# South-Twilight/ParallelWaveGAN

Hardware: AMD Instinct MI355X
Metric: audio samples/sec/GPU (24 kHz PWG, 80-band mel) + RTF at 1/2/4/8 MI355X (higher is better)
Workload: dtype f32 (fp16 hi+lo pair operands, 3 f16 MFMAs per product, fp32 accumulate); 1 GPU; libritts_v1 generator inference, 32 ragged utterances per GPU per step; model=ParallelWaveGANGenerator, hop=300, global_batch=32, frames_per_gpu=24295, parallelism=1 process, 1 GPU (no collective)

## Files before the change

### parallelwavegan_amd/csrc/pwg_capi.hip

```cpp
#include <hip/hip_runtime.h>

#include <algorithm>
#include <cmath>
#include <cstdio>
#include <cstdlib>
#include <cstring>
#include <map>
#include <mutex>
#include <string>
#include <utility>
#include <vector>

#include "../../include/pwg.h"
#include "pwg_internal.h"

#ifndef PWG_SMALL_SPREAD
#define PWG_SMALL_SPREAD 1
#endif

using namespace pwg;

namespace {

thread_local std::string g_err;
// ... 954 lines not shown
      give_back();
      return e;
    }
    h->records.push_back({bucket, a, b});
    return e;
  };

  int* range_flag = (int*)(ws + p->ws_flag);
  hipError_t e = hipSuccess;
  const int pipe_wg = h->n_cu / 8 * 8;
  const bool use_pipe = p->pipe_ok && h->layer_kernel == 3 && p->Tpad <= h->pipe_max && pipe_wg >= h->L;
  const bool split = h->layer_kernel == 2 || h->layer_kernel == 3;
  const bool split16 = h->layer_kernel == 3;
  const bool fuse_first = split16 && h->fuse_first && h->L > 1;
  UttDesc* d_utts = (UttDesc*)(ws + p->ws_utts);
  int* d_tile_utt = (int*)(ws + p->ws_tile_utt);
  long long* d_gap_col0 = (long long*)(ws + p->ws_gap);
  BlockDesc* d_blocks = (BlockDesc*)(ws + p->ws_blocks);
  for (int u0 = 0; u0 < p->n_utts; u0 += PLAN_CHUNK) {
    PlanDescArgs da;
    da.n = std::min(PLAN_CHUNK, p->n_utts - u0);
    da.u0 = u0;
    da.gap_tiles = (int)(h->gap / TILE);
    for (int i = 0; i < da.n; ++i) da.utts[i] = p->utts[u0 + i];
    da.d_utts = d_utts; da.tile_utt = d_tile_utt; da.gap_col0 = d_gap_col0; da.blocks = d_blocks;
    da.zero = u0 == 0 ? sched_ctr : nullptr;
    da.n_zero = (int)((p->ws_flag + sizeof(int) - p->ws_ctr) / sizeof(int));
    da.prog = use_pipe ? (int*)(ws + p->ws_prog) : nullptr;
    da.zx[0] = fuse_first ? reinterpret_cast<unsigned*>(x0) : nullptr;
    da.zx[1] = fuse_first ? reinterpret_cast<unsigned*>(x1) : nullptr;
    da.zx[2] = fuse_first && use_pipe ? reinterpret_cast<unsigned*>(ws + p->ws_x2) : nullptr;
    e = launch_plan_desc(da, p->max_blocks_per_utt, s);
    if (e != hipSuccess) return hip_fail(e, "plan descriptor launch");
  }
  ConvInArgs ca;
  ca.mel = mel; ca.mean = mean; ca.scale = scale; ca.w = packed + h->off_conv_in; ca.c1 = c1;
  ca.wfrag = packed + h->off_conv_in_frag;
  ca.utts = d_utts; ca.n_utts = p->n_utts; ca.F_total = p->F_total; ca.A = h->A; ca.KW = h->KW;
  ca.ctx = h->cfg.aux_context_window; ca.layout = p->layout; ca.use_conv_in = h->cfg.use_conv_in;
  e = timed(PWG_KERNEL_CONV_IN, [&] { return launch_conv_in(ca, s); });
  if (e != hipSuccess) return hip_fail(e, "conv_in launch");

  AuxProjArgs pa;
  pa.c1 = c1; pa.waux = packed + h->off_waux; pa.d = dproj; pa.F_total = p->F_total; pa.A = h->A; pa.GR = h->GR;
  pa.split = split16 ? 2 : split ? 1 : 0;
  pa.split_scale_a = (float)SPLIT_GATE_SCALE_TANH;
// ... 501 lines not shown
```

### parallelwavegan_amd/csrc/pwg_internal.h

```cpp
#pragma once
#include <hip/hip_runtime.h>
#include <stdint.h>

namespace pwg {

constexpr int TILE = 128;
constexpr int KC = 16;
constexpr int MAX_SCALES = 8;
constexpr int AUX_J4 = 8;
constexpr int AUX_MAX_NFWG = 16;

struct UttDesc {
  long long seg_base;
  long long first_tile;
  long long T;
  long long frame_base;
  long long frames;
  long long mel_off;
  long long io_off;
};

struct ConvInArgs {
  const float* mel;
  const float* mean;
// ... 63 lines not shown
  int R, RS, S, SS, KS;
  int dil;
  int nka;
  int nfwg;
  int tap_center;
  int first;
  const float* hw1;
  const float* hw2;
  const float* hb2;
  float* out;
  long long out_stride_t, out_stride_o;
  int O;
  float skip_scale;
};

struct BlockDesc {
  int col;
  int t0;
  int T;
  int frames;
  int frame_base;
  int io_off;
  int utt;
  int pad;
};

struct PersistArgs {
  const float* x_in;
  float* x_out;
  float* skip;
  const float* d;
  const float* tab;
  const BlockDesc* blocks;
  const float* wgp;
  const float* w2;
  const float* bg;
  const float* hw1;
  const float* hw2;
  const float* hb2;
  float* out;
  int tab_left, tab_right, tab_small;
  int H, J1, TL, TR, Fmin, nka;
  int n_blocks;
  int R, RS, S, SS, KS, dil, tap_center, first, O;
  int out_stride_t, out_stride_o;
  float skip_scale;
  int* ctr;
// ... 51 lines not shown
  unsigned* x[2];
  int* ctr;
  int l0, L;
  int half;
  int force_abort;
  int force_timeout;
  int waves_mid;
  int dil[PIPE_MAX_LAYERS];
};

constexpr int SCHED_CTR_STRIDE = 32;

int set_error(int code, const char* msg);

hipError_t allow_lds(const void* kfn, int lds);

constexpr int PLAN_CHUNK = 48;
constexpr int GAP_TILES_MAX = 1 << 20;
struct PlanDescArgs {
  UttDesc utts[PLAN_CHUNK];
  int n;
  int u0;
  int gap_tiles;
  UttDesc* d_utts;
  int* tile_utt;
  long long* gap_col0;
  BlockDesc* blocks;
  int* zero;
  int n_zero;
  int* prog;
  unsigned* zx[3];
};
hipError_t launch_plan_desc(const PlanDescArgs& a, long long max_blocks, hipStream_t s);

hipError_t launch_conv_in(const ConvInArgs& a, hipStream_t s);
hipError_t launch_aux_proj(const AuxProjArgs& a, int layers, hipStream_t s);
hipError_t launch_first_conv(const FirstConvArgs& a, long long n_tiles, hipStream_t s);
hipError_t launch_layer(const LayerArgs& a, int mt, int m2t, bool last, long long n_tiles, hipStream_t s);
hipError_t launch_first_conv_split(const FirstConvArgs& a, long long n_tiles, hipStream_t s);
hipError_t launch_first_conv_split16(const FirstConvArgs& a, long long n_tiles, hipStream_t s);
hipError_t launch_layer_split16(const SplitArgs& a, bool last, int tap_center, int waves_per_wg, int n_wg,
                                hipStream_t s, bool half = false);
hipError_t launch_layer_split(const SplitArgs& a, bool last, int tap_center, int waves_per_wg, int n_wg,
                              hipStream_t s);
hipError_t launch_pipe_split16(const PipeArgs& p, int tap_center, int n_wg, hipStream_t s);
hipError_t launch_sync_split16(const SyncArgs& p, int tap_center, int n_wg, hipStream_t s);
// ... 99 lines not shown
```

### parallelwavegan_amd/csrc/pwg_kernels.hip

```cpp
#include "pwg_internal.h"
#include "../../include/pwg.h"

namespace pwg {

typedef float f32x16 __attribute__((ext_vector_type(16)));
typedef float f32x4 __attribute__((ext_vector_type(4)));

__device__ __forceinline__ long long floordiv(long long a, long long b) {
  long long q = a / b;
  if ((a % b != 0) && (a < 0)) --q;
  return q;
}

__device__ __forceinline__ int find_utt_by_frame(const UttDesc* utts, int n, long long g) {
  int lo = 0, hi = n - 1;
  while (lo < hi) {
    int mid = (lo + hi + 1) >> 1;
    if (utts[mid].frame_base <= g) lo = mid; else hi = mid - 1;
  }
  return lo;
}

template <int OGMAX>
__global__ void __launch_bounds__(256) pwg_conv_in_kernel(const ConvInArgs a) {
// ... 833 lines not shown
      }
    }

    if (nblk < 0) break;
    blk = nblk;
    nblk = ticket_resolve(ticket);
  }
}

__global__ void __launch_bounds__(256) pwg_plan_desc_kernel(const PlanDescArgs a) {
  const int y = blockIdx.y;
  const UttDesc& d = a.utts[y];
  const long long j = (long long)blockIdx.x * 256 + threadIdx.x;
  const long long nb = (d.T + TILE - 1) / TILE * (TILE / 32);
  if (j < nb) {
    BlockDesc b;
    b.t0 = (int)(32 * j);
    b.col = (int)(d.seg_base + b.t0);
    b.T = (int)d.T;
    b.frames = (int)d.frames;
    b.frame_base = (int)d.frame_base;
    b.io_off = (int)d.io_off;
    b.utt = a.u0 + y;
    b.pad = 0;
    a.blocks[d.first_tile * (TILE / 32) + j] = b;
    if (a.prog != nullptr) a.prog[d.first_tile * (TILE / 32) + j] = 0;
    if ((j & (TILE / 32 - 1)) == 0) a.tile_utt[d.first_tile + j / (TILE / 32)] = a.u0 + y;
  }
  if (j < a.gap_tiles) {
    const long long seg_end = d.seg_base + (d.T + TILE - 1) / TILE * TILE;
    a.gap_col0[(long long)(a.u0 + y + 1) * a.gap_tiles + j] = seg_end + j * TILE;
    if (a.u0 == 0 && y == 0) a.gap_col0[j] = j * TILE;
  }
  if (j == 0) a.d_utts[a.u0 + y] = d;
  if (a.zero != nullptr && blockIdx.x == 0 && y == 0)
    for (int i = threadIdx.x; i < a.n_zero; i += 256) a.zero[i] = 0;
  if (a.zx[0] != nullptr && blockIdx.x == 0) {
    const long long seg_end = d.seg_base + (d.T + TILE - 1) / TILE * TILE;
    const int lead = a.u0 == 0 && y == 0 ? a.gap_tiles : 0;
    const int n4 = 64 * TILE / 4;
    typedef unsigned u32x4z __attribute__((ext_vector_type(4)));
    for (int t = 0; t < a.gap_tiles + lead; ++t) {
      const long long col0 = t < a.gap_tiles ? seg_end + (long long)t * TILE : (long long)(t - a.gap_tiles) * TILE;
#pragma unroll
      for (int pl = 0; pl < 3; ++pl) {
        if (a.zx[pl] == nullptr) continue;
        u32x4z* z = reinterpret_cast<u32x4z*>(a.zx[pl] + (size_t)col0 * 64);
// ... 112 lines not shown
```

### parallelwavegan_amd/csrc/pwg_split16.hip

```cpp
#include "pwg_internal.h"


namespace pwg {

namespace {

typedef float f32x4 __attribute__((ext_vector_type(4)));
typedef _Float16 f16x8 __attribute__((ext_vector_type(8)));
typedef unsigned u32x4 __attribute__((ext_vector_type(4)));

__device__ __forceinline__ f32x4 mma16(u32x4 a, u32x4 b, f32x4 c) {
  return __builtin_amdgcn_mfma_f32_16x16x32_f16(__builtin_bit_cast(f16x8, a), __builtin_bit_cast(f16x8, b), c, 0, 0,
                                                0);
}

__device__ __forceinline__ float gate16(float u, float v) {
  u = fminf(u, 64.f);
  const float e1 = __builtin_amdgcn_exp2f(u);
  const float e2 = __builtin_amdgcn_exp2f(v);
  return (1.f - e1) * __builtin_amdgcn_rcpf((1.f + e1) * (1.f + e2));
}

template <int NOPS>
__device__ __forceinline__ void split8x(const float (&v)[8], u32x4& hi, u32x4& lo) {
// ... 36 lines not shown
      "v_fma_mix_f32 %3, %22, %16, %3 op_sel:[1,0,0] op_sel_hi:[1,0,0]\n\t"
      "v_fma_mix_f32 %4, %23, %16, %4 op_sel_hi:[1,0,0]\n\t"
      "v_fma_mix_f32 %5, %23, %16, %5 op_sel:[1,0,0] op_sel_hi:[1,0,0]\n\t"
      "v_fma_mix_f32 %6, %24, %16, %6 op_sel_hi:[1,0,0]\n\t"
      "v_fma_mix_f32 %7, %24, %16, %7 op_sel:[1,0,0] op_sel_hi:[1,0,0]\n\t"
      "s_nop 1"
      : "=&v"(o[0]), "=&v"(o[1]), "=&v"(o[2]), "=&v"(o[3]), "=&v"(o[4]), "=&v"(o[5]), "=&v"(o[6]), "=&v"(o[7])
      : "v"(l[0]), "v"(l[1]), "v"(l[2]), "v"(l[3]), "v"(b0[0]), "v"(b0[1]), "v"(b0[2]), "v"(b0[3]), "v"(c),
        "v"(b1[0]), "v"(b1[1]), "v"(b1[2]), "v"(b1[3]), "v"(h[0]), "v"(h[1]), "v"(h[2]), "v"(h[3]));
}

struct Pair16 {
  unsigned hi, lo;
};
__device__ __forceinline__ Pair16 split_pair16(float v0, float v1) {
  typedef _Float16 f16x2 __attribute__((ext_vector_type(2)));
  const _Float16 h0 = (_Float16)v0, h1 = (_Float16)v1;
  const _Float16 l0 = (_Float16)(v0 - (float)h0), l1 = (_Float16)(v1 - (float)h1);
  return {__builtin_bit_cast(unsigned, f16x2{h0, h1}), __builtin_bit_cast(unsigned, f16x2{l0, l1})};
}

}

__device__ __forceinline__ size_t row16(int c, int g) {
  return (size_t)(c >> 5) * 2048 + (size_t)((c >> 4) & 1) * 1024 + (size_t)g * 64 + (size_t)(c & 15) * 4;
}

__device__ __forceinline__ unsigned row16_bytes(int c, int g) { return (unsigned)row16(c, g) * 4u; }

__device__ __forceinline__ __amdgpu_buffer_rsrc_t rsrc16(const void* base) {
  const unsigned long long b = (unsigned long long)base;
  const unsigned lo = __builtin_amdgcn_readfirstlane((unsigned)b), hi = __builtin_amdgcn_readfirstlane((unsigned)(b >> 32));
  return __builtin_amdgcn_make_buffer_rsrc((void*)(((unsigned long long)hi << 32) | lo), 0, 0x7fffffff, 0x00020000);
}
constexpr int AUX_SC1 = 16;
__device__ __forceinline__ u32x4 ld16_sc1(__amdgpu_buffer_rsrc_t r, unsigned off) {
  return __builtin_bit_cast(u32x4, __builtin_amdgcn_raw_buffer_load_b128(r, off, 0, AUX_SC1));
}
__device__ __forceinline__ void st16_sc1(__amdgpu_buffer_rsrc_t r, unsigned off, u32x4 v) {
  __builtin_amdgcn_raw_buffer_store_b128(v, r, off, 0, AUX_SC1);
}

struct Split16Smem {
  static constexpr int WG = 3 * 2 * 8 * 2 * 64 * 4;
  static constexpr int W2 = 2 * 8 * 2 * 64 * 4;
  static constexpr int BG = 8 * 16;
  static constexpr int BO = 64;
  static constexpr int HW1 = 4 * 4 * 64 * 4 + 64;
  static constexpr int dwords(bool last) { return WG + W2 + BG + BO + (last ? HW1 : 0); }
};
static_assert(Split16Smem::WG + Split16Smem::W2 + Split16Smem::BG + Split16Smem::BO == SPLIT_LAYER_DWORDS,
              "split16 layer image size");

template <bool LAST, bool FIRST>
__device__ __forceinline__ void s16_stage(const SplitArgs& a, unsigned* smem16) {
  const int nthr = blockDim.x;
  stage_lds(reinterpret_cast<u32x4*>(smem16), reinterpret_cast<const u32x4*>(a.wg), SPLIT_LAYER_DWORDS / 4,
            (int)threadIdx.x, nthr);
  if (LAST)
    stage_lds(reinterpret_cast<u32x4*>(smem16 + SPLIT_LAYER_DWORDS), reinterpret_cast<const u32x4*>(a.hw1),
              Split16Smem::HW1 / 4, (int)threadIdx.x, nthr);
  if (FIRST) {
    float* s_fwb = reinterpret_cast<float*>(smem16 + Split16Smem::dwords(LAST));
    for (int i = threadIdx.x; i < 128; i += nthr) s_fwb[i] = i < 64 ? a.fw[i] : a.fb[i - 64];
  }
}

template <int TC, bool FIRST, bool PIPE, int NTN = 2>
__device__ __forceinline__ void s16_bload(const SplitArgs& a, const float* s_fwb, const BlockDesc& d, int tap,
                                          u32x4 (&b)[8], int g, int c, int h16 = 0) {
  if constexpr (FIRST) {
    const f32x4* fw4 = reinterpret_cast<const f32x4*>(s_fwb) + g;
    const f32x4* fb4 = reinterpret_cast<const f32x4*>(s_fwb + 64) + g;
#pragma unroll
    for (int nt = 0; nt < NTN; ++nt) {
      const int t = d.t0 + h16 + 16 * nt + c + (tap - TC) * a.dil;
      const bool inside = t >= 0 && t < d.T;
      const float z = a.noise[d.io_off + (t < 0 ? 0 : (t >= d.T ? d.T - 1 : t))];
#pragma unroll
      for (int ks = 0; ks < 2; ++ks) {
        float v[8];
#pragma unroll
        for (int jh = 0; jh < 2; ++jh) {
          const f32x4 w = fw4[4 * (2 * ks + jh)], bb = fb4[4 * (2 * ks + jh)];
#pragma unroll
          for (int i = 0; i < 4; ++i) v[4 * jh + i] = inside ? fmaf(w[i], z, bb[i]) : 0.f;
        }
        split8x<0>(v, b[nt * 4 + ks * 2], b[nt * 4 + ks * 2 + 1]);
      }
    }
  } else if constexpr (PIPE) {
    const __amdgpu_buffer_rsrc_t r = rsrc16(a.x_in);
    const int cc = d.col + h16 + (tap - TC) * a.dil;
#pragma unroll
    for (int nt = 0; nt < NTN; ++nt) {
      const unsigned off = row16_bytes(cc + 16 * nt + c, g);
#pragma unroll
      for (int q = 0; q < 4; ++q) b[nt * 4 + q] = ld16_sc1(r, off + q * 1024u);
    }
  } else {
    const int cc = d.col + h16 + (tap - TC) * a.dil;
#pragma unroll
    for (int nt = 0; nt < NTN; ++nt) {
      const u32x4* p = reinterpret_cast<const u32x4*>(a.x_in + row16(cc + 16 * nt + c, g));
#pragma unroll
      for (int q = 0; q < 4; ++q) b[nt * 4 + q] = p[q * 64];
    }
  }
}

__device__ __forceinline__ void s16_load_dv(const SplitArgs& a, const BlockDesc& bd, unsigned (&dv)[2][8], int g,
                                            int c) {
  const int fw0 = bd.t0 / a.H - a.J1;
#pragma unroll
  for (int j = 0; j < 2; ++j) {
    const int f = fw0 + 2 * g + j;
    const int fc = f < 0 ? 0 : (f >= bd.frames ? bd.frames - 1 : f);
    const u32x4* drow = reinterpret_cast<const u32x4*>(a.d + (size_t)(bd.frame_base + fc) * 128 + 8 * c);
    const u32x4 d0 = drow[0], d1 = drow[1];
#pragma unroll
    for (int m = 0; m < 4; ++m) {
      dv[j][m] = d0[m];
      dv[j][m + 4] = d1[m];
    }
  }
}

template <bool PIPE, int NTN = 2>
__device__ __forceinline__ void s16_load_skip(const SplitArgs& a, const BlockDesc& bd, f32x4 (&sk)[4][2], int g,
                                              int c, int h16 = 0) {
  [[maybe_unused]] __amdgpu_buffer_rsrc_t rs;
  if constexpr (PIPE) rs = rsrc16(a.skip);
#pragma unroll
  for (int nt = 0; nt < NTN; ++nt)
#pragma unroll
    for (int ms = 0; ms < 4; ++ms) {
      if (a.first) {
        sk[ms][nt] = reinterpret_cast<const f32x4*>(a.skip0 + 16 * g)[ms];
      } else if constexpr (PIPE) {
        sk[ms][nt] = __builtin_bit_cast(f32x4, ld16_sc1(rs, row16_bytes(bd.col + h16 + 16 * nt + c, g) + ms * 1024u));
      } else {
        const f32x4* sp = reinterpret_cast<const f32x4*>(a.skip + row16(bd.col + h16 + 16 * nt + c, g));
        sk[ms][nt] = __builtin_nontemporal_load(sp + ms * 64);
      }
    }
}

template <bool LAST, int TC, bool FIRST, bool PIPE, int NTN = 2, typename Mid>
__device__ __forceinline__ void s16_block(const SplitArgs& a, const unsigned* smem16, const BlockDesc& bd,
                                          const BlockDesc& bdn, bool has_next, u32x4 (&b0)[8], u32x4 (&b1)[8],
                                          bool& nonfinite, Mid&& mid, int h16 = 0, int h16n = 0,
                                          bool poison = false) {
  static_assert(NTN == 2 || !LAST, "half blocks: middle layers");
  const unsigned* s_wg = smem16;
  const unsigned* s_w2 = s_wg + Split16Smem::WG;
  const unsigned* s_bg = s_w2 + Split16Smem::W2;
  const float* s_bo = reinterpret_cast<const float*>(s_bg + Split16Smem::BG);
  const float* s_hw1 = s_bo + Split16Smem::BO;
  const float* s_fwb = reinterpret_cast<const float*>(smem16 + Split16Smem::dwords(LAST));
  const int lane = threadIdx.x & 63;
  const int g = lane >> 4;
  const int c = lane & 15;
  constexpr int T1 = TC == 1 ? 2 : 1;
  const bool full = bd.t0 + h16 + 16 * NTN <= bd.T;

  unsigned dv[2][8];
  float bw[2][2];
#pragma unroll
  for (int nt = 0; nt < NTN; ++nt) {
    const int t = bd.t0 + h16 + 16 * nt + c;
    const bool live = t < bd.T;
    const int tc = live ? t : bd.T - 1;
    int roff;
    if (bd.frames < a.Fmin) roff = a.tab_small + (a.H * bd.frames * (bd.frames - 1) / 2 + tc) * AUX_J4;
    else if (tc < a.TL) roff = a.tab_left + tc * AUX_J4;
    else if (tc >= bd.T - a.TR) roff = a.tab_right + (bd.T - 1 - tc) * AUX_J4;
    else roff = (tc % a.H) * AUX_J4;
    const int shift = t / a.H - bd.t0 / a.H;
#pragma unroll
    for (int j = 0; j < 2; ++j) {
      const int idx = 2 * g + j - shift;
      const bool ok = live && idx >= 0 && idx < AUX_J4;
      const float w = a.tab[roff + (idx < 0 ? 0 : (idx >= AUX_J4 ? AUX_J4 - 1 : idx))];
      bw[nt][j] = ok ? w : 0.f;
    }
  }
  const u32x4* wgl = reinterpret_cast<const u32x4*>(s_wg) + lane;
  auto mma_tap = [&](f32x4 (&acc)[8][2], const u32x4 (&b)[8], int tap) {
#pragma unroll
    for (int ks = 0; ks < 2; ++ks) {
#pragma unroll
      for (int mh = 0; mh < 2; ++mh) {
        u32x4 ah[4], al[4];
#pragma unroll
        for (int mm = 0; mm < 4; ++mm) {
          const int m = 4 * mh + mm;
          ah[mm] = wgl[(((tap * 2 + ks) * 8 + m) * 2) * 64];
          al[mm] = wgl[(((tap * 2 + ks) * 8 + m) * 2 + 1) * 64];
        }
#pragma unroll
        for (int mm = 0; mm < 4; ++mm)
#pragma unroll
          for (int nt = 0; nt < NTN; ++nt) {
            f32x4& ac = acc[4 * mh + mm][nt];
            ac = mma16(ah[mm], b[nt * 4 + ks * 2], ac);
            ac = mma16(ah[mm], b[nt * 4 + ks * 2 + 1], ac);
            ac = mma16(al[mm], b[nt * 4 + ks * 2], ac);
          }
        __builtin_amdgcn_sched_barrier(0);
      }
    }
  };

  f32x4 acc[8][2];
#pragma unroll
  for (int m = 0; m < 8; ++m)
#pragma unroll
    for (int nt = 0; nt < NTN; ++nt) acc[m][nt] = f32x4{0.f, 0.f, 0.f, 0.f};
  f32x4 acc2[8][2];
  s16_bload<TC, FIRST, PIPE, NTN>(a, s_fwb, bd, T1, b1, g, c, h16);
  mma_tap(acc, b0, 0);
  s16_load_dv(a, bd, dv, g, c);
  s16_bload<TC, FIRST, PIPE, NTN>(a, s_fwb, bd, TC, b0, g, c, h16);
  mma_tap(acc, b1, T1);
  mma_tap(acc, b0, TC);
  if (!LAST) {
    const f32x4* bo_l = reinterpret_cast<const f32x4*>(s_bo + 16 * g);
#pragma unroll
    for (int nt = 0; nt < NTN; ++nt)
#pragma unroll
      for (int ks = 0; ks < 2; ++ks) {
        float o[8];
        seed8x(b0[nt * 4 + ks * 2], b0[nt * 4 + ks * 2 + 1], bo_l[2 * ks], bo_l[2 * ks + 1], 0.70710677f, o);
#pragma unroll
        for (int j = 0; j < 8; ++j) acc2[4 + 2 * ks + (j >> 2)][nt][j & 3] = o[j];
      }
  }
  mid();

  {
    f32x4 sk[4][2];
    s16_load_skip<PIPE, NTN>(a, bd, sk, g, c, h16);
#pragma unroll
    for (int nt = 0; nt < NTN; ++nt)
#pragma unroll
      for (int ms = 0; ms < 4; ++ms) acc2[ms][nt] = sk[ms][nt];
// ... 13 lines not shown
      const unsigned bgp = g == 0 ? bgl[16 * m] : 0u;
      const unsigned dh = __builtin_amdgcn_perm(dv[1][m], dv[0][m], 0x05040100u);
      const unsigned dl = __builtin_amdgcn_perm(dv[1][m], dv[0][m], 0x07060302u);
      const u32x4 aA = {dh, dl, dh, bgp};
#pragma unroll
      for (int nt = 0; nt < NTN; ++nt) acc[m][nt] = mma16(aA, bB[nt], acc[m][nt]);
    }
  }

  u32x4 gh[2][2], gl[2][2];
#pragma unroll
  for (int nt = 0; nt < NTN; ++nt)
#pragma unroll
    for (int ks = 0; ks < 2; ++ks) {
      float gv[8];
#pragma unroll
      for (int j = 0; j < 8; ++j) {
        const int m = 2 * ks + (j >> 2), i = j & 3;
        gv[j] = gate16(acc[m][nt][i], acc[m + 4][nt][i]);
      }
      split8x<0>(gv, gh[nt][ks], gl[nt][ks]);
    }

  if (has_next) s16_bload<TC, FIRST, PIPE, NTN>(a, s_fwb, bdn, 0, b0, g, c, h16n);
  constexpr int M2 = LAST ? 4 : 8;
  const u32x4* w2l = reinterpret_cast<const u32x4*>(s_w2) + lane;
#pragma unroll
  for (int ks = 0; ks < 2; ++ks)
#pragma unroll
    for (int mh = 0; mh < M2 / 4; ++mh) {
      u32x4 ah[4], al[4];
#pragma unroll
      for (int mm = 0; mm < 4; ++mm) {
        ah[mm] = w2l[((ks * 8 + 4 * mh + mm) * 2) * 64];
        al[mm] = w2l[((ks * 8 + 4 * mh + mm) * 2 + 1) * 64];
      }
#pragma unroll
      for (int mm = 0; mm < 4; ++mm)
#pragma unroll
        for (int nt = 0; nt < NTN; ++nt) {
          f32x4& ac = acc2[4 * mh + mm][nt];
          ac = mma16(ah[mm], gh[nt][ks], ac);
          ac = mma16(ah[mm], gl[nt][ks], ac);
          ac = mma16(al[mm], gh[nt][ks], ac);
        }
      __builtin_amdgcn_sched_barrier(0);
    }

  if (!LAST) {
    [[maybe_unused]] __amdgpu_buffer_rsrc_t rsk, rx;
    if constexpr (PIPE) {
      rsk = rsrc16(a.skip);
      rx = rsrc16(a.x_out);
    }
#pragma unroll
    for (int nt = 0; nt < NTN; ++nt) {
      const int col = bd.col + h16 + 16 * nt + c;
      const bool live = bd.t0 + h16 + 16 * nt + c < bd.T;
#pragma unroll
      for (int ms = 0; ms < 4; ++ms) {
        if constexpr (PIPE)
          st16_sc1(rsk, row16_bytes(col, g) + ms * 1024u, __builtin_bit_cast(u32x4, acc2[ms][nt]));
        else
          __builtin_nontemporal_store(acc2[ms][nt], reinterpret_cast<f32x4*>(a.skip + row16(col, g)) + ms * 64);
      }
#pragma unroll
      for (int ks = 0; ks < 2; ++ks) {
        float v[8];
#pragma unroll
        for (int j = 0; j < 8; ++j) v[j] = acc2[4 + 2 * ks + (j >> 2)][nt][j & 3];
        u32x4 vh, vl;
        split8x<11>(v, vh, vl);
        if (!full) {
#pragma unroll
          for (int k = 0; k < 4; ++k) {
            vh[k] = live ? vh[k] : 0u;
            vl[k] = live ? vl[k] : 0u;
          }
        }
        if constexpr (PIPE) {
          st16_sc1(rx, row16_bytes(col, g) + (ks * 2) * 1024u, vh);
          st16_sc1(rx, row16_bytes(col, g) + (ks * 2 + 1) * 1024u, vl);
        } else {
          u32x4* xp = reinterpret_cast<u32x4*>(a.x_out + row16(col, g));
          __builtin_nontemporal_store(vh, xp + (ks * 2) * 64);
          __builtin_nontemporal_store(vl, xp + (ks * 2 + 1) * 64);
        }
      }
    }
  } else {
    const u32x4* hw1 = reinterpret_cast<const u32x4*>(s_hw1) + lane;
    const f32x4* hb1 = reinterpret_cast<const f32x4*>(s_hw1 + 4 * 4 * 64 * 4 + 16 * g);
    f32x4 acc3[4][2];
#pragma unroll
    for (int m3 = 0; m3 < 4; ++m3)
#pragma unroll
      for (int nt = 0; nt < 2; ++nt) acc3[m3][nt] = hb1[m3];
    u32x4 sh[2][2], sl[2][2];
#pragma unroll
    for (int nt = 0; nt < 2; ++nt) {
      float sum = 0.f;
#pragma unroll
      for (int ms = 0; ms < 4; ++ms)
#pragma unroll
        for (int i = 0; i < 4; ++i) sum += acc2[ms][nt][i];
      nonfinite |= bd.t0 + 16 * nt + c < bd.T && !__builtin_isfinite(sum);
    }
#pragma unroll
    for (int nt = 0; nt < 2; ++nt)
#pragma unroll
// ... 22 lines not shown
      }
#pragma unroll
    for (int nt = 0; nt < 2; ++nt) {
      const int t = bd.t0 + 16 * nt + c;
      const bool live = t < bd.T;
      float* out = a.out + (size_t)bd.io_off * a.O + (size_t)t * a.out_stride_t;
      for (int oc = 0; oc < a.O; ++oc) {
        const f32x4* w = reinterpret_cast<const f32x4*>(a.hw2 + ((size_t)oc * 4 + g) * 16);
        float part = 0.f;
#pragma unroll
        for (int m3 = 0; m3 < 4; ++m3) {
          const f32x4 wq = w[m3];
#pragma unroll
          for (int i = 0; i < 4; ++i) part = fmaf(wq[i], fmaxf(acc3[m3][nt][i], 0.f), part);
        }
        part += __shfl_xor(part, 16);
        part += __shfl_xor(part, 32);
        if (g == 0 && live) out[(size_t)oc * a.out_stride_o] = poison ? __builtin_nanf("") : part + a.hb2[oc];
      }
    }
  }
}

template <bool LAST, int TC, bool FIRST, int NTN = 2>
__global__ void __launch_bounds__(512, 1) pwg_layer_split16_kernel(const SplitArgs a) {
  constexpr int UB = NTN == 1 ? 1 : 0;
  const int n_units = a.n_blocks << UB;
  extern __shared__ __attribute__((aligned(16))) unsigned smem16[];
  const bool tr = a.trace != nullptr;
  unsigned long long t_start = 0, c_start = 0, t_staged = 0, t_first = 0;
  if (tr) {
    t_start = __builtin_amdgcn_s_memrealtime();
    c_start = __builtin_amdgcn_s_memtime();
  }
  const int lane = threadIdx.x & 63;
  const int nw = a.compute_waves;
  const int xcd = blockIdx.x & 7;
  const int wave = threadIdx.x >> 6;
  const int blk0 = wave < nw ? (int)((long long)n_units * xcd / 8) + (blockIdx.x >> 3) * nw + wave : -1;
  bool poison = false;
  if constexpr (LAST)
    if (a.range_flag != nullptr)
      poison = (__hip_atomic_load(a.range_flag, __ATOMIC_RELAXED, __HIP_MEMORY_SCOPE_AGENT) & PWG_STATUS_REDO) != 0;
  const bool has0 = blk0 >= 0 && blk0 < (int)((long long)n_units * (xcd + 1) / 8);
  BlockDesc bdn;
  int h16n = 0;
  u32x4 b0[8], b1[8];
  if (has0) {
    bdn = a.blocks[blk0 >> UB];
    h16n = NTN == 1 ? 16 * (blk0 & 1) : 0;
    if constexpr (!FIRST) s16_bload<TC, false, false, NTN>(a, nullptr, bdn, 0, b0, lane >> 4, lane & 15, h16n);
  }
  s16_stage<LAST, FIRST>(a, smem16);
  __syncthreads();
  int n_done = 0;
  auto trace_out = [&]() {
    if (tr && lane == 0) {
      unsigned long long* r = a.trace + ((size_t)blockIdx.x * (blockDim.x >> 6) + wave) * 8;
      const unsigned long long t_end = __builtin_amdgcn_s_memrealtime(), c_end = __builtin_amdgcn_s_memtime();
      r[0] = t_start; r[1] = t_staged; r[2] = t_first; r[3] = t_end; r[4] = (unsigned long long)n_done;
      r[5] = c_start; r[6] = c_end; r[7] = (unsigned long long)__builtin_amdgcn_s_getreg((20 << 0) | (0 << 6) | (3 << 11));
    }
  };
  if (tr) t_staged = __builtin_amdgcn_s_memrealtime();
  if (wave >= nw) {
    trace_out();
    return;
  }
  auto xcd_waves = [&](int y) { return (((int)gridDim.x - y + 7) >> 3) * nw; };
  auto xcd_first = [&](int y) { return (int)((long long)n_units * y / 8); };
  const int x_first = xcd_first(xcd), x_end = xcd_first(xcd + 1), x_waves = xcd_waves(xcd);
  int victim = 0;
  auto ticket_issue = [&]() -> int {
    int v = 0;
// ... 7 lines not shown
      if (i < x_end) return i;
      victim = 1;
    }
    for (; victim < 8; ++victim) {
      const int y = (xcd + victim) & 7;
      int tk = 0;
      if (lane == 0)
        tk = __hip_atomic_fetch_add(a.ctr + y * SCHED_CTR_STRIDE, 1, __ATOMIC_RELAXED, __HIP_MEMORY_SCOPE_AGENT);
      const int i = xcd_first(y) + 2 * xcd_waves(y) + __builtin_amdgcn_readfirstlane(tk);
      if (i < xcd_first(y + 1)) return i;
    }
    return -1;
  };

  int blk = x_first + (blockIdx.x >> 3) * nw + wave;
  int nblk = blk + x_waves;
  if (blk >= x_end) blk = -1;
  if (nblk >= x_end) nblk = -1;
  if (blk < 0) {
    trace_out();
    return;
  }
  const float* s_fwb = reinterpret_cast<const float*>(smem16 + Split16Smem::dwords(LAST));
  if constexpr (FIRST) s16_bload<TC, true, false, NTN>(a, s_fwb, bdn, 0, b0, lane >> 4, lane & 15, h16n);
  bool nonfinite = false;
  while (true) {
    const BlockDesc bd = bdn;
    const int h16 = h16n;
    const int pf = nblk >= 0 ? nblk : blk;
    bdn = a.blocks[pf >> UB];
    h16n = NTN == 1 ? 16 * (pf & 1) : 0;
    int ticket = 0;
    s16_block<LAST, TC, FIRST, false, NTN>(a, smem16, bd, bdn, true, b0, b1, nonfinite, [&]() {
      if (nblk >= 0) ticket = ticket_issue();
    }, h16, h16n, poison);
    if (tr && n_done++ == 0) t_first = __builtin_amdgcn_s_memrealtime();
    if (nblk < 0) break;
    blk = nblk;
    nblk = ticket_resolve(ticket);
  }
  if (LAST && nonfinite && a.range_flag) flag_status(a.range_flag, a.sticky, PWG_STATUS_RANGE);
  trace_out();
}

constexpr int PIPE_SPIN_LIMIT = 1 << 20;

template <bool LAST, int TC, bool FIRST>
__device__ __forceinline__ void pipe_layer(const PipeArgs& p, int l, unsigned* smem16) {
  SplitArgs a = p.base;
  a.wg = p.wg0 + (size_t)l * p.wg_stride;
  a.d = p.d0 + (size_t)l * p.d_stride;
  a.x_in = p.x[l % 3];
  a.x_out = p.x[(l + 1) % 3];
  a.dil = p.dil[l];
  a.first = l == 0;
  if (!FIRST) a.noise = nullptr;
// ... 15 lines not shown
    const int i = lane - left, bb = b + i;
    const bool need = lane <= left + right && bb >= 0 && bb < a.n_blocks;
    const int thr = (i >= -rl1 && i <= rr1) ? l : l - 1;
    for (int spins = 0;; ++spins) {
      const int v = need ? __hip_atomic_load(p.prog + (need ? bb : 0), __ATOMIC_RELAXED, __HIP_MEMORY_SCOPE_AGENT)
                         : 0x7fffffff;
      if (__all(v >= thr)) break;
      if (spins >= PIPE_SPIN_LIMIT) {
        if (lane == 0) flag_status(p.base.range_flag, p.base.sticky, PWG_STATUS_PIPE_TIMEOUT);
        break;
      }
      __builtin_amdgcn_s_sleep(2);
    }
    __builtin_amdgcn_fence(__ATOMIC_ACQUIRE, "wavefront");
  };

  bool nonfinite = false;
  const float* s_fwb = reinterpret_cast<const float*>(smem16 + Split16Smem::dwords(LAST));
  int blk = ticket();
  u32x4 b0[8], b1[8];
  while (blk < a.n_blocks) {
    const BlockDesc bd = a.blocks[blk];
    wait_deps(blk);
    s16_bload<TC, FIRST, true>(a, s_fwb, bd, 0, b0, lane >> 4, lane & 15);
    int next = 0;
    s16_block<LAST, TC, FIRST, true>(a, smem16, bd, bd, false, b0, b1, nonfinite, [&]() { next = ticket(); });
    if (!LAST) {
      asm volatile("s_waitcnt vmcnt(0)" ::: "memory");
      if (lane == 0) __hip_atomic_store(p.prog + blk, l + 1, __ATOMIC_RELAXED, __HIP_MEMORY_SCOPE_AGENT);
    }
    blk = next;
  }
  if (LAST && nonfinite && a.range_flag) flag_status(a.range_flag, a.sticky, PWG_STATUS_RANGE);
}

template <int TC>
__global__ void __launch_bounds__(512, 1) pwg_pipe_split16_kernel(const PipeArgs p) {
  extern __shared__ __attribute__((aligned(16))) unsigned smem16[];
  const int nwg = gridDim.x;
  const int lin = (blockIdx.x & 7) * (nwg >> 3) + (blockIdx.x >> 3);
  const int l = (int)((long long)lin * p.L / nwg);
  if (l == p.L - 1) pipe_layer<true, TC, false>(p, l, smem16);
  else if (l == 0 && p.base.noise != nullptr) pipe_layer<false, TC, true>(p, l, smem16);
  else pipe_layer<false, TC, false>(p, l, smem16);
}

template <int TC, bool FIRST, int NTN>
__device__ __forceinline__ void sync_layer(const SplitArgs& a, const unsigned* smem16) {
  constexpr int UB = NTN == 1 ? 1 : 0;
  const int n_units = a.n_blocks << UB;
  const int nw = a.compute_waves;
  const int wave = threadIdx.x >> 6;
  if (wave >= nw) return;
  const int lane = threadIdx.x & 63;
  const int xcd = blockIdx.x & 7;
  const int x_first = (int)((long long)n_units * xcd / 8), x_end = (int)((long long)n_units * (xcd + 1) / 8);
  const int x_waves = (((int)gridDim.x - xcd + 7) >> 3) * nw;
  int u = x_first + (blockIdx.x >> 3) * nw + wave;
  if (u >= x_end) return;
  const float* s_fwb = reinterpret_cast<const float*>(smem16 + Split16Smem::dwords(false));
  bool nonfinite = false;
  BlockDesc bd = a.blocks[u >> UB];
  int h16 = NTN == 1 ? 16 * (u & 1) : 0;
  u32x4 b0[8], b1[8];
  s16_bload<TC, FIRST, true, NTN>(a, s_fwb, bd, 0, b0, lane >> 4, lane & 15, h16);
  while (true) {
    const int un = u + x_waves;
    const bool has_next = un < x_end;
    const BlockDesc bdn = a.blocks[(has_next ? un : u) >> UB];
    const int h16n = NTN == 1 ? 16 * ((has_next ? un : u) & 1) : 0;
    s16_block<false, TC, FIRST, true, NTN>(a, smem16, bd, bdn, has_next, b0, b1, nonfinite, []() {}, h16, h16n);
    if (!has_next) break;
    u = un;
    bd = bdn;
    h16 = h16n;
  }
}

constexpr int SYNC_RESIDENCY_SPINS = 512;

template <int TC, int NTN>
__global__ void __launch_bounds__(512, 1) pwg_sync_split16_kernel(const SyncArgs p) {
  extern __shared__ __attribute__((aligned(16))) unsigned smem16[];
  __shared__ int s_decision;
  const int nwg = gridDim.x;
  int* const bar = p.ctr;
  int* const arrive = p.ctr + SCHED_CTR_STRIDE;
  int* const decision = p.ctr + 2 * SCHED_CTR_STRIDE;
// ... 105 lines not shown
      for (int e = 0; e < 2; ++e) {
        const int j = 2 * dw + e;
        const int ch = 16 * (2 * ks + (j >> 2)) + 4 * g + (j & 3);
        y[e] = fmaf(a.w[ch], z, a.b[ch]);
      }
      const Pair16 pr = split_pair16(y[0], y[1]);
      v = hl ? pr.lo : pr.hi;
    }
    x[(size_t)col0 * 64 + idx] = v;
  }
}

hipError_t launch_first_conv_split16(const FirstConvArgs& a, long long n_tiles, hipStream_t s) {
  hipLaunchKernelGGL(pwg_first_conv_split16_kernel, dim3((unsigned)n_tiles), dim3(256), 0, s, a);
  return hipGetLastError();
}

hipError_t launch_layer_split16(const SplitArgs& a, bool last, int tap_center, int waves_per_wg, int n_wg,
                                hipStream_t s, bool half) {
  if (waves_per_wg > 8) waves_per_wg = 8;
  if (a.compute_waves < 1 || a.compute_waves > waves_per_wg) return hipErrorInvalidValue;
  if (half && last) return hipErrorInvalidValue;
  const dim3 grid((unsigned)n_wg), block((unsigned)(64 * waves_per_wg));
#define PWG_SPLIT16_LAUNCH(LAST_, TC_, FIRST_, NTN_)                                                    \
  {                                                                                                     \
    const size_t lds = sizeof(unsigned) * (Split16Smem::dwords(LAST_) + (FIRST_ ? 128 : 0));            \
    auto kfn = &pwg_layer_split16_kernel<LAST_, TC_, FIRST_, NTN_>;                                     \
    hipError_t e_ = allow_lds(reinterpret_cast<const void*>(kfn), (int)lds);                           \
    if (e_ != hipSuccess) return e_;                                                                    \
    hipLaunchKernelGGL(kfn, grid, block, lds, s, a);                                                    \
    return hipGetLastError();                                                                           \
  }
  const bool first = a.noise != nullptr;
  if (first && last) return hipErrorInvalidValue;
  if (tap_center == 1) {
    if (half) {
      if (first) PWG_SPLIT16_LAUNCH(false, 1, true, 1) else PWG_SPLIT16_LAUNCH(false, 1, false, 1)
    }
    if (first) PWG_SPLIT16_LAUNCH(false, 1, true, 2)
    if (last) PWG_SPLIT16_LAUNCH(true, 1, false, 2) else PWG_SPLIT16_LAUNCH(false, 1, false, 2)
  } else if (tap_center == 2) {
    if (half) {
      if (first) PWG_SPLIT16_LAUNCH(false, 2, true, 1) else PWG_SPLIT16_LAUNCH(false, 2, false, 1)
    }
    if (first) PWG_SPLIT16_LAUNCH(false, 2, true, 2)
    if (last) PWG_SPLIT16_LAUNCH(true, 2, false, 2) else PWG_SPLIT16_LAUNCH(false, 2, false, 2)
  }
#undef PWG_SPLIT16_LAUNCH
  return hipErrorInvalidValue;
}

hipError_t launch_sync_split16(const SyncArgs& p, int tap_center, int n_wg, hipStream_t s) {
  const size_t lds = sizeof(unsigned) * (Split16Smem::dwords(false) + 128);
  if (p.L < 1 || p.L > PIPE_MAX_LAYERS || p.waves_mid < 1 || p.waves_mid > 8) return hipErrorInvalidValue;
  if (n_wg < 8) return hipErrorInvalidValue;
  auto kfn = tap_center == 1 ? (p.half ? &pwg_sync_split16_kernel<1, 1> : &pwg_sync_split16_kernel<1, 2>)
             : tap_center == 2 ? (p.half ? &pwg_sync_split16_kernel<2, 1> : &pwg_sync_split16_kernel<2, 2>)
                               : nullptr;
  if (kfn == nullptr) return hipErrorInvalidValue;
  const hipError_t e = allow_lds(reinterpret_cast<const void*>(kfn), (int)lds);
  if (e != hipSuccess) return e;
  hipLaunchKernelGGL(kfn, dim3((unsigned)n_wg), dim3(512), lds, s, p);
  return hipGetLastError();
}

hipError_t launch_pipe_split16(const PipeArgs& p, int tap_center, int n_wg, hipStream_t s) {
  const size_t lds = sizeof(unsigned) * (Split16Smem::dwords(true) > Split16Smem::dwords(false) + 128
                                             ? Split16Smem::dwords(true) : Split16Smem::dwords(false) + 128);
  if (n_wg < p.L || n_wg % 8 != 0) return hipErrorInvalidValue;
  auto kfn = tap_center == 1 ? &pwg_pipe_split16_kernel<1> : tap_center == 2 ? &pwg_pipe_split16_kernel<2> : nullptr;
// ... 9 lines not shown
```

Baseline: 148.2 million audio samples/s (whole job, all GPUs).

## Cut address arithmetic in split16 layer kernel via scalar offsets and precomputed frame index

Precomputes each block's frame index (t0/H) in the plan descriptor and replaces per-lane integer division with a wrap test when H is at least 32. Block descriptors are made wave-uniform with readfirstlane, so scalar base offsets go into SGPRs and buffer-load soffset while per-lane offsets stay small 32-bit values. Adds a template variant for dilations that are multiples of 16, which skips the shifted-row address computation. The aim is to lower VALU address math and VGPR pressure in the inner loop, at the cost of more kernel instantiations and reliance on the descriptor values being uniform.

```diff
diff --git a/parallelwavegan_amd/csrc/pwg_capi.hip b/parallelwavegan_amd/csrc/pwg_capi.hip
--- a/parallelwavegan_amd/csrc/pwg_capi.hip
+++ b/parallelwavegan_amd/csrc/pwg_capi.hip
@@ -1000,6 +1000,7 @@
     da.n = std::min(PLAN_CHUNK, p->n_utts - u0);
     da.u0 = u0;
     da.gap_tiles = (int)(h->gap / TILE);
+    da.H = (int)h->aux.H;
     for (int i = 0; i < da.n; ++i) da.utts[i] = p->utts[u0 + i];
     da.d_utts = d_utts; da.tile_utt = d_tile_utt; da.gap_col0 = d_gap_col0; da.blocks = d_blocks;
     da.zero = u0 == 0 ? sched_ctr : nullptr;
diff --git a/parallelwavegan_amd/csrc/pwg_internal.h b/parallelwavegan_amd/csrc/pwg_internal.h
--- a/parallelwavegan_amd/csrc/pwg_internal.h
+++ b/parallelwavegan_amd/csrc/pwg_internal.h
@@ -109,7 +109,7 @@
   int frame_base;
   int io_off;
   int utt;
-  int pad;
+  int f0;
 };
 
 struct PersistArgs {
@@ -207,6 +207,7 @@
   int n;
   int u0;
   int gap_tiles;
+  int H;
   UttDesc* d_utts;
   int* tile_utt;
   long long* gap_col0;
diff --git a/parallelwavegan_amd/csrc/pwg_kernels.hip b/parallelwavegan_amd/csrc/pwg_kernels.hip
--- a/parallelwavegan_amd/csrc/pwg_kernels.hip
+++ b/parallelwavegan_amd/csrc/pwg_kernels.hip
@@ -879,7 +879,7 @@
     b.frame_base = (int)d.frame_base;
     b.io_off = (int)d.io_off;
     b.utt = a.u0 + y;
-    b.pad = 0;
+    b.f0 = b.t0 / a.H;
     a.blocks[d.first_tile * (TILE / 32) + j] = b;
     if (a.prog != nullptr) a.prog[d.first_tile * (TILE / 32) + j] = 0;
     if ((j & (TILE / 32 - 1)) == 0) a.tile_utt[d.first_tile + j / (TILE / 32)] = a.u0 + y;
diff --git a/parallelwavegan_amd/csrc/pwg_split16.hip b/parallelwavegan_amd/csrc/pwg_split16.hip
--- a/parallelwavegan_amd/csrc/pwg_split16.hip
+++ b/parallelwavegan_amd/csrc/pwg_split16.hip
@@ -82,11 +82,23 @@
 
 }
 
-__device__ __forceinline__ size_t row16(int c, int g) {
-  return (size_t)(c >> 5) * 2048 + (size_t)((c >> 4) & 1) * 1024 + (size_t)g * 64 + (size_t)(c & 15) * 4;
-}
-
-__device__ __forceinline__ unsigned row16_bytes(int c, int g) { return (unsigned)row16(c, g) * 4u; }
+__device__ __forceinline__ unsigned shifted16(int r, int g, int c) {
+  const unsigned s = (unsigned)(r + c);
+  return (unsigned)g * 256u + (s >> 4) * 4096u + (s & 15u) * 16u;
+}
+
+__device__ __forceinline__ BlockDesc uniform_desc(const BlockDesc& d) {
+  BlockDesc u;
+  u.col = __builtin_amdgcn_readfirstlane(d.col);
+  u.t0 = __builtin_amdgcn_readfirstlane(d.t0);
+  u.T = __builtin_amdgcn_readfirstlane(d.T);
+  u.frames = __builtin_amdgcn_readfirstlane(d.frames);
+  u.frame_base = __builtin_amdgcn_readfirstlane(d.frame_base);
+  u.io_off = __builtin_amdgcn_readfirstlane(d.io_off);
+  u.utt = __builtin_amdgcn_readfirstlane(d.utt);
+  u.f0 = __builtin_amdgcn_readfirstlane(d.f0);
+  return u;
+}
 
 __device__ __forceinline__ __amdgpu_buffer_rsrc_t rsrc16(const void* base) {
   const unsigned long long b = (unsigned long long)base;
@@ -94,12 +106,33 @@
   return __builtin_amdgcn_make_buffer_rsrc((void*)(((unsigned long long)hi << 32) | lo), 0, 0x7fffffff, 0x00020000);
 }
 constexpr int AUX_SC1 = 16;
-__device__ __forceinline__ u32x4 ld16_sc1(__amdgpu_buffer_rsrc_t r, unsigned off) {
-  return __builtin_bit_cast(u32x4, __builtin_amdgcn_raw_buffer_load_b128(r, off, 0, AUX_SC1));
-}
-__device__ __forceinline__ void st16_sc1(__amdgpu_buffer_rsrc_t r, unsigned off, u32x4 v) {
-  __builtin_amdgcn_raw_buffer_store_b128(v, r, off, 0, AUX_SC1);
-}
+
+template <bool PIPE>
+struct Plane16 {
+  char* p;
+  __amdgpu_buffer_rsrc_t r;
+  __device__ __forceinline__ explicit Plane16(const void* base) : p(const_cast<char*>(static_cast<const char*>(base))) {
+    if constexpr (PIPE) r = rsrc16(base);
+  }
+  __device__ __forceinline__ char* at(long long sb) const {
+    asm("" : "+s"(sb));
+    return p + sb;
+  }
+  template <bool NT = false>
+  __device__ __forceinline__ u32x4 load(long long sb, unsigned vo, int imm) const {
+    if constexpr (PIPE) {
+      return __builtin_bit_cast(u32x4, __builtin_amdgcn_raw_buffer_load_b128(r, vo + (unsigned)imm, (unsigned)sb, AUX_SC1));
+    } else {
+      const u32x4* q = reinterpret_cast<const u32x4*>(at(sb) + imm + (size_t)vo);
+      if constexpr (NT) return __builtin_nontemporal_load(q);
+      else return *q;
+    }
+  }
+  __device__ __forceinline__ void store(long long sb, unsigned vo, int imm, u32x4 v) const {
+    if constexpr (PIPE) __builtin_amdgcn_raw_buffer_store_b128(v, r, vo + (unsigned)imm, (unsigned)sb, AUX_SC1);
+    else __builtin_nontemporal_store(v, reinterpret_cast<u32x4*>(at(sb) + imm + (size_t)vo));
+  }
+};
 
 struct Split16Smem {
   static constexpr int WG = 3 * 2 * 8 * 2 * 64 * 4;
@@ -126,17 +159,20 @@
   }
 }
 
-template <int TC, bool FIRST, bool PIPE, int NTN = 2>
+template <int TC, bool FIRST, bool PIPE, int NTN = 2, bool AL = false>
 __device__ __forceinline__ void s16_bload(const SplitArgs& a, const float* s_fwb, const BlockDesc& d, int tap,
                                           u32x4 (&b)[8], int g, int c, int h16 = 0) {
   if constexpr (FIRST) {
     const f32x4* fw4 = reinterpret_cast<const f32x4*>(s_fwb) + g;
     const f32x4* fb4 = reinterpret_cast<const f32x4*>(s_fwb + 64) + g;
+    const char* nz = reinterpret_cast<const char*>(a.noise + d.io_off);
+    const int ts = d.t0 + h16 + (tap - TC) * a.dil;
 #pragma unroll
     for (int nt = 0; nt < NTN; ++nt) {
-      const int t = d.t0 + h16 + 16 * nt + c + (tap - TC) * a.dil;
+      const int t = ts + 16 * nt + c;
       const bool inside = t >= 0 && t < d.T;
-      const float z = a.noise[d.io_off + (t < 0 ? 0 : (t >= d.T ? d.T - 1 : t))];
+      const unsigned tcl = (unsigned)(t < 0 ? 0 : (t >= d.T ? d.T - 1 : t));
+      const float z = *reinterpret_cast<const float*>(nz + (size_t)(tcl * 4u));
 #pragma unroll
       for (int ks = 0; ks < 2; ++ks) {
         float v[8];
@@ -149,34 +185,27 @@
         split8x<0>(v, b[nt * 4 + ks * 2], b[nt * 4 + ks * 2 + 1]);
       }
     }
-  } else if constexpr (PIPE) {
-    const __amdgpu_buffer_rsrc_t r = rsrc16(a.x_in);
-    const int cc = d.col + h16 + (tap - TC) * a.dil;
-#pragma unroll
-    for (int nt = 0; nt < NTN; ++nt) {
-      const unsigned off = row16_bytes(cc + 16 * nt + c, g);
-#pragma unroll
-      for (int q = 0; q < 4; ++q) b[nt * 4 + q] = ld16_sc1(r, off + q * 1024u);
-    }
   } else {
     const int cc = d.col + h16 + (tap - TC) * a.dil;
-#pragma unroll
-    for (int nt = 0; nt < NTN; ++nt) {
-      const u32x4* p = reinterpret_cast<const u32x4*>(a.x_in + row16(cc + 16 * nt + c, g));
-#pragma unroll
-      for (int q = 0; q < 4; ++q) b[nt * 4 + q] = p[q * 64];
-    }
+    const long long sb = (long long)(cc >> 4) * 4096;
+    const unsigned vo = (AL || tap == TC) ? 16u * (unsigned)(16 * g + c) : shifted16(cc & 15, g, c);
+    const Plane16<PIPE> x(a.x_in);
+#pragma unroll
+    for (int nt = 0; nt < NTN; ++nt)
+#pragma unroll
+      for (int q = 0; q < 4; ++q) b[nt * 4 + q] = x.load(sb + nt * 4096, vo, q * 1024);
   }
 }
 
 __device__ __forceinline__ void s16_load_dv(const SplitArgs& a, const BlockDesc& bd, unsigned (&dv)[2][8], int g,
                                             int c) {
-  const int fw0 = bd.t0 / a.H - a.J1;
+  const int fw0 = bd.f0 - a.J1;
+  const char* dbase = reinterpret_cast<const char*>(a.d + (size_t)bd.frame_base * 128);
 #pragma unroll
   for (int j = 0; j < 2; ++j) {
     const int f = fw0 + 2 * g + j;
     const int fc = f < 0 ? 0 : (f >= bd.frames ? bd.frames - 1 : f);
-    const u32x4* drow = reinterpret_cast<const u32x4*>(a.d + (size_t)(bd.frame_base + fc) * 128 + 8 * c);
+    const u32x4* drow = reinterpret_cast<const u32x4*>(dbase + (size_t)((unsigned)fc * 512u + (unsigned)c * 32u));
     const u32x4 d0 = drow[0], d1 = drow[1];
 #pragma unroll
     for (int m = 0; m < 4; ++m) {
@@ -189,29 +218,26 @@
 template <bool PIPE, int NTN = 2>
 __device__ __forceinline__ void s16_load_skip(const SplitArgs& a, const BlockDesc& bd, f32x4 (&sk)[4][2], int g,
                                               int c, int h16 = 0) {
-  [[maybe_unused]] __amdgpu_buffer_rsrc_t rs;
-  if constexpr (PIPE) rs = rsrc16(a.skip);
+  const Plane16<PIPE> skip(a.skip);
+  const long long sb = (long long)((bd.col + h16) >> 4) * 4096;
+  const unsigned vo = 16u * (unsigned)(16 * g + c);
 #pragma unroll
   for (int nt = 0; nt < NTN; ++nt)
 #pragma unroll
     for (int ms = 0; ms < 4; ++ms) {
-      if (a.first) {
-        sk[ms][nt] = reinterpret_cast<const f32x4*>(a.skip0 + 16 * g)[ms];
-      } else if constexpr (PIPE) {
-        sk[ms][nt] = __builtin_bit_cast(f32x4, ld16_sc1(rs, row16_bytes(bd.col + h16 + 16 * nt + c, g) + ms * 1024u));
-      } else {
-        const f32x4* sp = reinterpret_cast<const f32x4*>(a.skip + row16(bd.col + h16 + 16 * nt + c, g));
-        sk[ms][nt] = __builtin_nontemporal_load(sp + ms * 64);
-      }
-    }
-}
-
-template <bool LAST, int TC, bool FIRST, bool PIPE, int NTN = 2, typename Mid>
-__device__ __forceinline__ void s16_block(const SplitArgs& a, const unsigned* smem16, const BlockDesc& bd,
-                                          const BlockDesc& bdn, bool has_next, u32x4 (&b0)[8], u32x4 (&b1)[8],
-                                          bool& nonfinite, Mid&& mid, int h16 = 0, int h16n = 0,
+      if (a.first) sk[ms][nt] = reinterpret_cast<const f32x4*>(a.skip0 + 16 * g)[ms];
+      else sk[ms][nt] = __builtin_bit_cast(f32x4, skip.template load<true>(sb + nt * 4096, vo, ms * 1024));
+    }
+}
+
+template <bool LAST, int TC, bool FIRST, bool PIPE, int NTN = 2, bool AL = false, typename Mid>
+__device__ __forceinline__ void s16_block(const SplitArgs& a, const unsigned* smem16, const BlockDesc& bd_v,
+                                          const BlockDesc& bdn_v, bool has_next, u32x4 (&b0)[8], u32x4 (&b1)[8],
+                                          bool& nonfinite, Mid&& mid, int h16_v = 0, int h16n_v = 0,
                                           bool poison = false) {
   static_assert(NTN == 2 || !LAST, "half blocks: middle layers");
+  const BlockDesc bd = uniform_desc(bd_v);
+  const int h16 = NTN == 1 ? __builtin_amdgcn_readfirstlane(h16_v) : 0;
   const unsigned* s_wg = smem16;
   const unsigned* s_w2 = s_wg + Split16Smem::WG;
   const unsigned* s_bg = s_w2 + Split16Smem::W2;
@@ -226,22 +252,35 @@
 
   unsigned dv[2][8];
   float bw[2][2];
+  const bool two_frames = a.H >= 32;
+  const int rem0 = bd.t0 - bd.f0 * a.H;
 #pragma unroll
   for (int nt = 0; nt < NTN; ++nt) {
-    const int t = bd.t0 + h16 + 16 * nt + c;
+    const int x = h16 + 16 * nt + c;
+    const int t = bd.t0 + x;
     const bool live = t < bd.T;
     const int tc = live ? t : bd.T - 1;
+    int shift, rem;
+    if (two_frames) {
+      const int r = rem0 + x;
+      const bool wrap = r >= a.H;
+      shift = wrap ? 1 : 0;
+      rem = wrap ? r - a.H : r;
+    } else {
+      shift = t / a.H - bd.t0 / a.H;
+      rem = tc % a.H;
+    }
     int roff;
     if (bd.frames < a.Fmin) roff = a.tab_small + (a.H * bd.frames * (bd.frames - 1) / 2 + tc) * AUX_J4;
     else if (tc < a.TL) roff = a.tab_left + tc * AUX_J4;
     else if (tc >= bd.T - a.TR) roff = a.tab_right + (bd.T - 1 - tc) * AUX_J4;
-    else roff = (tc % a.H) * AUX_J4;
-    const int shift = t / a.H - bd.t0 / a.H;
+    else roff = rem * AUX_J4;
 #pragma unroll
     for (int j = 0; j < 2; ++j) {
       const int idx = 2 * g + j - shift;
       const bool ok = live && idx >= 0 && idx < AUX_J4;
-      const float w = a.tab[roff + (idx < 0 ? 0 : (idx >= AUX_J4 ? AUX_J4 - 1 : idx))];
+      const unsigned e = (unsigned)(roff + (idx < 0 ? 0 : (idx >= AUX_J4 ? AUX_J4 - 1 : idx)));
+      const float w = *reinterpret_cast<const float*>(reinterpret_cast<const char*>(a.tab) + (size_t)(e * 4u));
       bw[nt][j] = ok ? w : 0.f;
     }
   }
@@ -278,10 +317,10 @@
 #pragma unroll
     for (int nt = 0; nt < NTN; ++nt) acc[m][nt] = f32x4{0.f, 0.f, 0.f, 0.f};
   f32x4 acc2[8][2];
-  s16_bload<TC, FIRST, PIPE, NTN>(a, s_fwb, bd, T1, b1, g, c, h16);
+  s16_bload<TC, FIRST, PIPE, NTN, AL>(a, s_fwb, bd, T1, b1, g, c, h16);
   mma_tap(acc, b0, 0);
   s16_load_dv(a, bd, dv, g, c);
-  s16_bload<TC, FIRST, PIPE, NTN>(a, s_fwb, bd, TC, b0, g, c, h16);
+  s16_bload<TC, FIRST, PIPE, NTN, AL>(a, s_fwb, bd, TC, b0, g, c, h16);
   mma_tap(acc, b1, T1);
   mma_tap(acc, b0, TC);
   if (!LAST) {
@@ -341,7 +380,11 @@
       split8x<0>(gv, gh[nt][ks], gl[nt][ks]);
     }
 
-  if (has_next) s16_bload<TC, FIRST, PIPE, NTN>(a, s_fwb, bdn, 0, b0, g, c, h16n);
+  if (has_next) {
+    const BlockDesc bdn = uniform_desc(bdn_v);
+    const int h16n = NTN == 1 ? __builtin_amdgcn_readfirstlane(h16n_v) : 0;
+    s16_bload<TC, FIRST, PIPE, NTN, AL>(a, s_fwb, bdn, 0, b0, g, c, h16n);
+  }
   constexpr int M2 = LAST ? 4 : 8;
   const u32x4* w2l = reinterpret_cast<const u32x4*>(s_w2) + lane;
 #pragma unroll
@@ -367,22 +410,15 @@
     }
 
   if (!LAST) {
-    [[maybe_unused]] __amdgpu_buffer_rsrc_t rsk, rx;
-    if constexpr (PIPE) {
-      rsk = rsrc16(a.skip);
-      rx = rsrc16(a.x_out);
-    }
+    const Plane16<PIPE> skip(a.skip), xo(a.x_out);
+    const long long sb = (long long)((bd.col + h16) >> 4) * 4096;
+    const unsigned vo = 16u * (unsigned)lane;
 #pragma unroll
     for (int nt = 0; nt < NTN; ++nt) {
-      const int col = bd.col + h16 + 16 * nt + c;
       const bool live = bd.t0 + h16 + 16 * nt + c < bd.T;
 #pragma unroll
-      for (int ms = 0; ms < 4; ++ms) {
-        if constexpr (PIPE)
-          st16_sc1(rsk, row16_bytes(col, g) + ms * 1024u, __builtin_bit_cast(u32x4, acc2[ms][nt]));
-        else
-          __builtin_nontemporal_store(acc2[ms][nt], reinterpret_cast<f32x4*>(a.skip + row16(col, g)) + ms * 64);
-      }
+      for (int ms = 0; ms < 4; ++ms)
+        skip.store(sb + nt * 4096, vo, ms * 1024, __builtin_bit_cast(u32x4, acc2[ms][nt]));
 #pragma unroll
       for (int ks = 0; ks < 2; ++ks) {
         float v[8];
@@ -397,14 +433,8 @@
             vl[k] = live ? vl[k] : 0u;
           }
         }
-        if constexpr (PIPE) {
-          st16_sc1(rx, row16_bytes(col, g) + (ks * 2) * 1024u, vh);
-          st16_sc1(rx, row16_bytes(col, g) + (ks * 2 + 1) * 1024u, vl);
-        } else {
-          u32x4* xp = reinterpret_cast<u32x4*>(a.x_out + row16(col, g));
-          __builtin_nontemporal_store(vh, xp + (ks * 2) * 64);
-          __builtin_nontemporal_store(vl, xp + (ks * 2 + 1) * 64);
-        }
+        xo.store(sb + nt * 4096, vo, (ks * 2) * 1024, vh);
+        xo.store(sb + nt * 4096, vo, (ks * 2 + 1) * 1024, vl);
       }
     }
   } else {
@@ -473,7 +503,7 @@
   }
 }
 
-template <bool LAST, int TC, bool FIRST, int NTN = 2>
+template <bool LAST, int TC, bool FIRST, bool AL, int NTN>
 __global__ void __launch_bounds__(512, 1) pwg_layer_split16_kernel(const SplitArgs a) {
   constexpr int UB = NTN == 1 ? 1 : 0;
   const int n_units = a.n_blocks << UB;
@@ -500,7 +530,9 @@
   if (has0) {
     bdn = a.blocks[blk0 >> UB];
     h16n = NTN == 1 ? 16 * (blk0 & 1) : 0;
-    if constexpr (!FIRST) s16_bload<TC, false, false, NTN>(a, nullptr, bdn, 0, b0, lane >> 4, lane & 15, h16n);
+    if constexpr (!FIRST)
+      s16_bload<TC, false, false, NTN, AL>(a, nullptr, uniform_desc(bdn), 0, b0, lane >> 4, lane & 15,
+                                           NTN == 1 ? __builtin_amdgcn_readfirstlane(h16n) : 0);
   }
   s16_stage<LAST, FIRST>(a, smem16);
   __syncthreads();
@@ -554,7 +586,9 @@
     return;
   }
   const float* s_fwb = reinterpret_cast<const float*>(smem16 + Split16Smem::dwords(LAST));
-  if constexpr (FIRST) s16_bload<TC, true, false, NTN>(a, s_fwb, bdn, 0, b0, lane >> 4, lane & 15, h16n);
+  if constexpr (FIRST)
+    s16_bload<TC, true, false, NTN>(a, s_fwb, uniform_desc(bdn), 0, b0, lane >> 4, lane & 15,
+                                    NTN == 1 ? __builtin_amdgcn_readfirstlane(h16n) : 0);
   bool nonfinite = false;
   while (true) {
     const BlockDesc bd = bdn;
@@ -563,7 +597,7 @@
     bdn = a.blocks[pf >> UB];
     h16n = NTN == 1 ? 16 * (pf & 1) : 0;
     int ticket = 0;
-    s16_block<LAST, TC, FIRST, false, NTN>(a, smem16, bd, bdn, true, b0, b1, nonfinite, [&]() {
+    s16_block<LAST, TC, FIRST, false, NTN, AL>(a, smem16, bd, bdn, true, b0, b1, nonfinite, [&]() {
       if (nblk >= 0) ticket = ticket_issue();
     }, h16, h16n, poison);
     if (tr && n_done++ == 0) t_first = __builtin_amdgcn_s_memrealtime();
@@ -625,7 +659,7 @@
   while (blk < a.n_blocks) {
     const BlockDesc bd = a.blocks[blk];
     wait_deps(blk);
-    s16_bload<TC, FIRST, true>(a, s_fwb, bd, 0, b0, lane >> 4, lane & 15);
+    s16_bload<TC, FIRST, true>(a, s_fwb, uniform_desc(bd), 0, b0, lane >> 4, lane & 15);
     int next = 0;
     s16_block<LAST, TC, FIRST, true>(a, smem16, bd, bd, false, b0, b1, nonfinite, [&]() { next = ticket(); });
     if (!LAST) {
@@ -653,7 +687,7 @@
   constexpr int UB = NTN == 1 ? 1 : 0;
   const int n_units = a.n_blocks << UB;
   const int nw = a.compute_waves;
-  const int wave = threadIdx.x >> 6;
+  const int wave = __builtin_amdgcn_readfirstlane(threadIdx.x >> 6);
   if (wave >= nw) return;
   const int lane = threadIdx.x & 63;
   const int xcd = blockIdx.x & 7;
@@ -666,7 +700,8 @@
   BlockDesc bd = a.blocks[u >> UB];
   int h16 = NTN == 1 ? 16 * (u & 1) : 0;
   u32x4 b0[8], b1[8];
-  s16_bload<TC, FIRST, true, NTN>(a, s_fwb, bd, 0, b0, lane >> 4, lane & 15, h16);
+  s16_bload<TC, FIRST, true, NTN>(a, s_fwb, uniform_desc(bd), 0, b0, lane >> 4, lane & 15,
+                                  NTN == 1 ? __builtin_amdgcn_readfirstlane(h16) : 0);
   while (true) {
     const int un = u + x_waves;
     const bool has_next = un < x_end;
@@ -818,10 +853,10 @@
   if (a.compute_waves < 1 || a.compute_waves > waves_per_wg) return hipErrorInvalidValue;
   if (half && last) return hipErrorInvalidValue;
   const dim3 grid((unsigned)n_wg), block((unsigned)(64 * waves_per_wg));
-#define PWG_SPLIT16_LAUNCH(LAST_, TC_, FIRST_, NTN_)                                                    \
+#define PWG_SPLIT16_LAUNCH(LAST_, TC_, FIRST_, NTN_, AL_)                                               \
   {                                                                                                     \
     const size_t lds = sizeof(unsigned) * (Split16Smem::dwords(LAST_) + (FIRST_ ? 128 : 0));            \
-    auto kfn = &pwg_layer_split16_kernel<LAST_, TC_, FIRST_, NTN_>;                                     \
+    auto kfn = &pwg_layer_split16_kernel<LAST_, TC_, FIRST_, AL_, NTN_>;                                \
     hipError_t e_ = allow_lds(reinterpret_cast<const void*>(kfn), (int)lds);                           \
     if (e_ != hipSuccess) return e_;                                                                    \
     hipLaunchKernelGGL(kfn, grid, block, lds, s, a);                                                    \
@@ -829,19 +864,23 @@
   }
   const bool first = a.noise != nullptr;
   if (first && last) return hipErrorInvalidValue;
+  const bool al = a.dil % 16 == 0;
+#define PWG_SPLIT16_MIDDLE(TC_, NTN_) \
+  { if (al) PWG_SPLIT16_LAUNCH(false, TC_, false, NTN_, true) else PWG_SPLIT16_LAUNCH(false, TC_, false, NTN_, false) }
   if (tap_center == 1) {
     if (half) {
-      if (first) PWG_SPLIT16_LAUNCH(false, 1, true, 1) else PWG_SPLIT16_LAUNCH(false, 1, false, 1)
-    }
-    if (first) PWG_SPLIT16_LAUNCH(false, 1, true, 2)
-    if (last) PWG_SPLIT16_LAUNCH(true, 1, false, 2) else PWG_SPLIT16_LAUNCH(false, 1, false, 2)
+      if (first) PWG_SPLIT16_LAUNCH(false, 1, true, 1, false) else PWG_SPLIT16_MIDDLE(1, 1)
+    }
+    if (first) PWG_SPLIT16_LAUNCH(false, 1, true, 2, false)
+    if (last) PWG_SPLIT16_LAUNCH(true, 1, false, 2, false) else PWG_SPLIT16_MIDDLE(1, 2)
   } else if (tap_center == 2) {
     if (half) {
-      if (first) PWG_SPLIT16_LAUNCH(false, 2, true, 1) else PWG_SPLIT16_LAUNCH(false, 2, false, 1)
-    }
-    if (first) PWG_SPLIT16_LAUNCH(false, 2, true, 2)
-    if (last) PWG_SPLIT16_LAUNCH(true, 2, false, 2) else PWG_SPLIT16_LAUNCH(false, 2, false, 2)
-  }
+      if (first) PWG_SPLIT16_LAUNCH(false, 2, true, 1, false) else PWG_SPLIT16_MIDDLE(2, 1)
+    }
+    if (first) PWG_SPLIT16_LAUNCH(false, 2, true, 2, false)
+    if (last) PWG_SPLIT16_LAUNCH(true, 2, false, 2, false) else PWG_SPLIT16_MIDDLE(2, 2)
+  }
+#undef PWG_SPLIT16_MIDDLE
 #undef PWG_SPLIT16_LAUNCH
   return hipErrorInvalidValue;
 }
```

Result: faster. 151.9 million audio samples/s (whole job, all GPUs), median of 6 (+2.5%).
